# rishabhjain16/audio-visual-llm

Hardware: AMD Instinct MI355X
Metric: AV-clip train-step samples/sec (clip_whisper -> Llama-2-7B LoRA), whole job (higher is better)
Workload: dtype bf16

## Files before the change

audio-visual-llm_amd/csrc/api.hip:

```cpp
#include "common.h"
#include "avllm_internal.h"
#include <stdarg.h>

static thread_local char g_err[512] = "";

int av_set_error(int code, const char* fmt, ...) {
    va_list ap;
    va_start(ap, fmt);
    vsnprintf(g_err, sizeof(g_err), fmt, ap);
    va_end(ap);
    return code;
}

#include <mutex>
#include <string.h>
static const struct { const char* name; int dflt; } g_knob_def[AV_KNOB_COUNT] = {
    {"DECODE_FUSED", 1}, {"DEC_AL", 0}, {"LORA_UNBATCHED", 0}, {"F8_UNFUSED_QUANT", 0}, {"F8_FAST", 1}, {"ATTN_SHORT", 1},
    {"NARROW_EPILOGUE", 0}, {"TN_CHUNK", 0}, {"GEMM_DBG", 0}, {"GEMM_GW", 0}, {"GEMM_VARIANT", 0}};
static int g_knob[AV_KNOB_COUNT];
static std::once_flag g_knob_once;
static void knob_init() {
    for (int i = 0; i < AV_KNOB_COUNT; ++i) {
        char env[64];
        snprintf(env, sizeof(env), "AVLLM_%s", g_knob_def[i].name);
        const char* e = getenv(env);
        g_knob[i] = e ? atoi(e) : g_knob_def[i].dflt;
    }
}
int av_knob(int id) {
    std::call_once(g_knob_once, knob_init);
    return g_knob[id];
}
static int* knob_slot(const char* name) {
    std::call_once(g_knob_once, knob_init);
    for (int i = 0; name && i < AV_KNOB_COUNT; ++i)
        if (!strcmp(name, g_knob_def[i].name)) return &g_knob[i];
    return nullptr;
}

int av_device(int* ncu) {
    static int g_ncu[AV_MAX_DEVICES];
    int dev = 0;
    if (hipGetDevice(&dev) != hipSuccess) dev = 0;
    const int slot = dev & (AV_MAX_DEVICES - 1);
    if (!g_ncu[slot] && hipDeviceGetAttribute(&g_ncu[slot], hipDeviceAttributeMultiprocessorCount, dev) != hipSuccess) g_ncu[slot] = 256;
    *ncu = g_ncu[slot];
    return slot;
}

#define ST ((hipStream_t)stream)
extern "C" {
int avllm_set_knob(const char* name, int32_t value) {
    int* k = knob_slot(name);
    AV_CHECK_ARG(k, "set_knob: unknown knob '%s'", name ? name : "(null)");
    *k = value;
    return AV_OK;
}
int avllm_get_knob(const char* name, int32_t* value) {
    const int* k = knob_slot(name);
    AV_CHECK_ARG(k && value, "get_knob: unknown knob '%s'", name ? name : "(null)");
    *value = *k;
    return AV_OK;
}
int avllm_set_gemm_variant(int v) { return avllm_set_knob("GEMM_VARIANT", v); }
const char* avllm_last_error(void) { return g_err; }
int avllm_version(void) { return 100; }

int avllm_gemm(const avllm_gemm_desc* d, void* stream) { return av_gemm(d, ST); }
int avllm_gemm_plan(const avllm_gemm_desc* d, int32_t* kernel) { AV_CHECK_ARG(kernel, "gemm_plan: null kernel"); return av_gemm_plan(d, kernel); }
int avllm_gemm_tn(const void* P, int64_t ldp, int32_t I, const void* Q, int64_t ldq, int32_t J, int32_t M, float* out,
                  int64_t ldo, float alpha, int32_t dtype, void* stream) { return av_gemm_tn(P, ldp, I, Q, ldq, J, M, out, ldo, alpha, dtype, ST); }
int avllm_gemm_tn_drop(const void* P, int64_t ldp, int32_t I, const void* Q, int64_t ldq, int32_t J, int32_t M, float* out,
                       int64_t ldo, float alpha, uint32_t seed, float p, int32_t dtype, void* stream) { return av_gemm_tn(P, ldp, I, Q, ldq, J, M, out, ldo, alpha, dtype, ST, seed, p); }
int avllm_layernorm(const void* x, const void* w, const void* b, void* y, int64_t rows, int32_t d, float eps, int32_t dtype,
                    void* stream) { return av_layernorm(x, w, b, y, rows, d, eps, dtype, ST); }
int avllm_rmsnorm_fwd(const void* x, const void* w, void* y, float* rstd, int64_t rows, int32_t d, float eps, int32_t dtype,
                      void* stream) { return av_rmsnorm_fwd(x, w, y, rstd, rows, d, eps, dtype, ST); }
int avllm_rmsnorm_bwd(const void* dy, const void* x, const void* w, const float* rstd, const void* dres_in, void* dx_out,
                      int64_t rows, int32_t d, int32_t dtype, void* stream) { return av_rmsnorm_bwd(dy, x, w, rstd, dres_in, dx_out, rows, d, dtype, ST); }
int avllm_rope(void* x, int64_t ld, int64_t rows, int32_t T, int32_t heads, int32_t hd, int32_t pos0, float theta,
               int32_t inverse, int32_t dtype, void* stream) { return av_rope(x, ld, rows, T, heads, hd, pos0, theta, inverse, dtype, ST); }
int avllm_rope_table(float* tab, int32_t T, int32_t hd, int32_t pos0, float theta, const int32_t* pos_dev, float factor,
                     float low_freq_factor, float high_freq_factor, int32_t orig_ctx, void* stream) {
    AvRopeScale sc;
    sc.factor = factor; sc.low_freq_factor = low_freq_factor; sc.high_freq_factor = high_freq_factor; sc.orig_ctx = orig_ctx;
    AV_CHECK_ARG(orig_ctx <= 0 || (factor > 0.f && low_freq_factor > 0.f && high_freq_factor > low_freq_factor), "rope_table: bad llama3 scaling");
    return av_rope_table(tab, T, hd, pos0, theta, ST, pos_dev, sc);
}
int avllm_rope_tab(void* x, int64_t ld, int64_t rows, int32_t T, int32_t heads, int32_t hd, const float* tab, int32_t inverse,
                   int32_t dtype, void* stream) { return av_rope_tab(x, ld, rows, T, heads, hd, tab, inverse, dtype, ST); }
int avllm_kv_append(const void* k, const void* v, int64_t ld, void* kc, void* vc, int32_t B, int32_t T, int32_t pos0, int32_t Tmax,
                    int32_t d, int32_t dtype, void* stream) { return av_kv_append(k, v, ld, kc, vc, B, T, pos0, Tmax, d, dtype, ST); }
int avllm_swiglu_fwd(const void* gu, void* h, int64_t M, int32_t F, int32_t dtype, void* stream) { return av_swiglu_fwd(gu, h, M, F, dtype, ST); }
int avllm_swiglu_bwd(const void* dh, const void* gu, void* dgu, int64_t M, int32_t F, int32_t dtype, void* stream) { return av_swiglu_bwd(dh, gu, dgu, M, F, dtype, ST); }
int avllm_attention_fwd(const void* q, const void* k, const void* v, void* o, float* lse, int32_t B, int32_t Tq, int32_t Tk,
                        int32_t H, int32_t hd, int64_t ldq, int64_t ldk, int64_t ldv, int64_t ldo, float scale, int32_t causal,
                        int32_t dtype, int32_t impl, int32_t kv_heads, void* stream) {
    return av_attention_fwd(q, k, v, o, lse, B, Tq, Tk, H, hd, ldq, ldk, ldv, ldo, scale, causal, dtype, impl, ST, kv_heads);
}
int avllm_attention_bwd(const void* q, const void* k, const void* v, const void* o, const void* dout, const float* lse, void* dq,
                        void* dk, void* dv, float* delta_ws, int32_t B, int32_t T, int32_t H, int32_t hd, int64_t ldq, int64_t ldk,
                        int64_t ldv, int64_t ldo, int64_t lddq, int64_t lddk, int64_t lddv, float scale, int32_t causal,
                        int32_t dtype, int32_t impl, int32_t kv_heads, void* stream) {
    return av_attention_bwd(q, k, v, o, dout, lse, dq, dk, dv, delta_ws, B, T, H, hd, ldq, ldk, ldv, ldo, lddq, lddk, lddv, scale, causal, dtype, impl, ST, kv_heads);
}
int avllm_ce_fwd(const void* logits, int64_t ld, const int64_t* labels, int32_t B, int32_t T, int32_t V, float* row_lse,
                 float* loss_sum, float* count, int32_t dtype, void* stream) { return av_ce_fwd(logits, ld, labels, B, T, V, row_lse, loss_sum, count, dtype, ST); }
int avllm_ce_bwd(const void* logits, int64_t ld, const int64_t* labels, const float* row_lse, const float* count, float grad_scale,
                 void* dlogits, int32_t B, int32_t T, int32_t V, int32_t dtype, void* stream) { return av_ce_bwd(logits, ld, labels, row_lse, count, grad_scale, dlogits, B, T, V, dtype, ST); }
int avllm_argmax_rows(const void* logits, int64_t ld, int64_t rows, int32_t V, int64_t* out, int32_t dtype, void* stream) { return av_argmax_rows(logits, ld, rows, V, out, dtype, ST); }
int avllm_sample_rows(const void* logits, int64_t ld, int64_t rows, int32_t V, float temperature, int32_t top_k, float top_p, uint32_t seed,
                      const uint32_t* row_seeds, int32_t step, const int32_t* step_dev, uint8_t* unfinished, int64_t eos, int64_t pad,
                      int64_t* out, int32_t dtype, void* stream) {
    return av_sample_rows(logits, ld, rows, V, temperature, top_k, top_p, seed, row_seeds, step, step_dev, unfinished, eos, pad, out, dtype, ST);
}
size_t avllm_beam_topk_workspace_bytes(int64_t rows, int32_t V, int32_t k) { return av_beam_topk_workspace_bytes(rows, V, k); }
int avllm_beam_topk(const float* logits, int64_t ld, int32_t B, int32_t num_beams, int32_t V, const float* beam_scores, int32_t k,
                    float* out_scores, int32_t* out_beams, int64_t* out_tokens, void* ws, size_t ws_bytes, void* stream) {
    return av_beam_topk(logits, ld, B, num_beams, V, beam_scores, k, out_scores, out_beams, out_tokens, ws, ws_bytes, 0, ST);
}
int avllm_beam_topk_logprobs(const float* logprobs, int64_t ld, int32_t B, int32_t num_beams, int32_t V, const float* beam_scores, int32_t k,
                             float* out_scores, int32_t* out_beams, int64_t* out_tokens, void* ws, size_t ws_bytes, void* stream) {
    return av_beam_topk(logprobs, ld, B, num_beams, V, beam_scores, k, out_scores, out_beams, out_tokens, ws, ws_bytes, 1, ST);
}
int avllm_logits_process(void* scores, int64_t ld, int64_t rows, int32_t V, int64_t* history, int64_t ldh, const int64_t* append, int32_t cur,
                         const int32_t* cur_dev, float repetition_penalty, int32_t no_repeat_ngram_size, int32_t min_new_tokens, int64_t eos,
                         int32_t log_softmax, int32_t dtype, void* stream) {
    return av_logits_process(scores, ld, rows, V, history, ldh, append, cur, cur_dev, repetition_penalty, no_repeat_ngram_size, min_new_tokens, eos,
                             log_softmax, dtype, ST);
}
int avllm_kv_gather_rows(const void* k_src, const void* v_src, int32_t src_rows, int64_t src_T, void* k_dst, void* v_dst, int32_t dst_rows,
                         int64_t dst_T, int32_t layers, int32_t dkv, const int32_t* parent, int32_t t0, int32_t t1, int32_t dtype, void* stream) {
    return av_kv_gather_rows(k_src, v_src, src_rows, src_T, k_dst, v_dst, dst_rows, dst_T, layers, dkv, parent, t0, t1, dtype, ST);
}
int avllm_embedding(const void* table, const int64_t* ids, void* out, int64_t n, int32_t d, int32_t dtype, void* stream) { return av_embedding(table, ids, out, n, d, dtype, ST); }
int avllm_cast(const void* src, int32_t sdt, void* dst, int32_t ddt, int64_t n, void* stream) { return av_cast(src, sdt, dst, ddt, n, ST); }
int avllm_dropout(const void* x, void* y, int64_t rows, int32_t d, uint32_t seed, float p, int32_t dtype, void* stream) { return av_dropout(x, y, rows, d, seed, p, dtype, ST); }
int avllm_whisper_im2col1(const float* mel, void* cols, int32_t B, int32_t n_mels, int32_t T, int32_t Kpad, int32_t dtype, void* stream) { return av_whisper_im2col1(mel, cols, B, n_mels, T, Kpad, dtype, ST); }
int avllm_whisper_im2col2(const void* h, void* cols, int32_t B, int32_t T, int32_t d, int32_t dtype, void* stream) { return av_whisper_im2col2(h, cols, B, T, d, dtype, ST); }
int avllm_clip_patchify(const float* frames, void* cols, int32_t N, int32_t S, int32_t p, int32_t Kpad, int32_t dtype, void* stream) { return av_clip_patchify(frames, cols, N, S, p, Kpad, dtype, ST); }
int avllm_clip_cls_rows(const void* ce, const void* pos, void* x, int32_t N, int32_t tokens, int32_t d, int32_t dtype, void* stream) { return av_clip_cls_rows(ce, pos, x, N, tokens, d, dtype, ST); }
int avllm_fuse_pool(const void* a, int32_t Ta, const void* v, int32_t Tv, const void* pe, int32_t P, void* out, int32_t B, int32_t L,
                    int32_t S_out, int32_t D, float fs, int32_t dtype, void* stream) { return av_fuse_pool(a, Ta, v, Tv, pe, P, out, B, L, S_out, D, fs, dtype, ST); }
int avllm_fuse_pool_bwd(const void* dx, void* da, int32_t Ta, void* dv, int32_t Tv, int32_t P, int32_t B, int32_t L, int32_t S_out, int32_t D,
                        float fs, int32_t dtype, void* stream) { return av_fuse_pool_bwd(dx, da, Ta, dv, Tv, P, B, L, S_out, D, fs, dtype, ST); }
int avllm_gemm_wgrad(const void* dY, int64_t ldy, const void* X, int64_t ldx, int32_t M, int32_t N, int32_t K, float* dW, int64_t ldw, float* db,
                     float alpha, int32_t dtype, void* stream) { return av_gemm_wgrad(dY, ldy, X, ldx, M, N, K, dW, ldw, db, alpha, dtype, ST); }
int avllm_grad_sumsq_det_multi(const float* const* g, const int64_t* n, int32_t nbuf, float* partials, int32_t nparts, float* sumsq, void* stream) {
    return av_grad_sumsq_det_multi(g, n, nbuf, partials, nparts, sumsq, ST);
}
int avllm_adamw_step_multi(const avllm_adamw_seg* segs, int32_t nseg, float lr, float b1, float b2, float eps, int32_t step, const float* sumsq,
                           float max_norm, float prescale, const float* guard, float* skipped, const avllm_step_state* state, void* stream) {
    return av_adamw_step_multi(segs, nseg, lr, b1, b2, eps, step, sumsq, max_norm, prescale, guard, skipped, state, ST);
}
int avllm_grad_sumsq(const float* g, int64_t n, float* sumsq, void* stream) { return av_grad_sumsq(g, n, sumsq, ST); }
int avllm_grad_sumsq_det(const float* g, int64_t n, float* partials, int32_t nparts, float* sumsq, void* stream) { return av_grad_sumsq_det(g, n, partials, nparts, sumsq, ST); }
int avllm_adamw_step(float* p, const float* g, float* m, float* v, int64_t n, float lr, float b1, float b2, float eps, float wd,
                     int32_t step, const float* sumsq, float max_norm, float prescale, const float* guard, float* skipped,
                     const avllm_step_state* state, void* stream) {
    return av_adamw_step(p, g, m, v, n, lr, b1, b2, eps, wd, step, sumsq, max_norm, prescale, guard, skipped, state, ST);
}
int avllm_act_residual(const void* x, const void* r, void* y, int64_t n, int32_t act, int32_t dtype, void* stream) { return av_act_residual(x, r, y, n, act, dtype, ST); }
int avllm_step_advance(avllm_step_state* state, const avllm_schedule* sched, void* stream) { return av_step_advance(state, sched, ST); }
int avllm_lora_pack(const float* A, const float* Bm, int32_t r, int32_t din, int32_t dout, void* A_pad, void* AT_pad, int64_t ld_at,
                    void* B_pad, void* BT_pad, int32_t dtype, void* stream) { return av_lora_pack(A, Bm, r, din, dout, A_pad, AT_pad, ld_at, B_pad, BT_pad, dtype, ST); }
}
```

audio-visual-llm_amd/csrc/attention.hip:

```cpp
#include "common.h"
#include "avllm_internal.h"
#include <type_traits>
#include <cstdlib>

int av_attention_fwd_ref(const void* q, const void* k, const void* v, void* o, float* lse, int B, int Tq, int Tk, int H,
                         int hd, long ldq, long ldk, long ldv, long ldo, float scale, int causal, int dtype, hipStream_t st, int G);
int av_attention_delta(const void* o, const void* dout, float* delta, int B, int T, int H, int hd, long ldo, long lddo, int dtype, hipStream_t st);
int av_attention_bwd_ref(const void* q, const void* k, const void* v, const void* dout, const float* lse, const float* delta,
                         void* dq, void* dk, void* dv, int B, int T, int H, int hd, long ldq, long ldk, long ldv, long lddo,
                         long lddq, long lddk, long lddv, float scale, int causal, int dtype, hipStream_t st, int G);
int av_attention_bwd_mfma(const void* q, const void* k, const void* v, const void* dout, const float* lse, float* delta,
                          void* dq, void* dk, void* dv, int B, int T, int H, int hd, long ldq, long ldk, long ldv, long lddo,
                          long lddq, long lddk, long lddv, float scale, int causal, hipStream_t st, int G, const void* o, long ldo, const float* rope_tab);

namespace {

typedef __attribute__((address_space(3))) short4v* lds_s4_ptr;

__device__ __forceinline__ int acc_row(int reg, int half) { return (reg & 3) + 8 * (reg >> 2) + 4 * half; }
__device__ __forceinline__ float max3f(float a, float x, float y) { return __builtin_elementwise_maximum(__builtin_elementwise_maximum(a, x), y); }

template <int HD, int NW, bool CAUSAL>
__global__ __launch_bounds__(NW * 64, 2) void attn_fwd_mfma(const bf16* __restrict__ q, const bf16* __restrict__ k,
                                                         const bf16* __restrict__ v, bf16* __restrict__ o, float* __restrict__ lse,
// ... 75 lines not shown
            }
        }
        __syncthreads();
    }
    auto park = [&](int buf) {
#pragma unroll
        for (int i = 0; i < NCH; ++i) {
            const int c = tid + i * NT;
            if (c < 64 * CPR) {
                const int row = c / CPR, ch = c % CPR;
                *(u32x4*)(k_lds_ + buf * LROWS * KS + row * KS + ch * 16) = kreg[i];
                *(u32x4*)(v_lds_ + buf * LROWS * VS + row * VS + ch * 16) = vreg[i];
            }
        }
    };
    if (PREFETCH) prefetch(0);
    if (DB) { park(0); if (64 < k_end) prefetch(64); }
    for (int kb = 0; kb < k_end; kb += 64) {
        const int lrow0 = ONESHOT ? kb : 0;
        if (DB) {
            const int buf = (kb >> 6) & 1;
            __syncthreads();
            if (kb + 64 < k_end) { park(buf ^ 1); if (kb + 128 < k_end) prefetch(kb + 128); }
            k_lds = k_lds_ + buf * LROWS * KS; v_lds = v_lds_ + buf * LROWS * VS;
        } else if (!ONESHOT) {
            if (!PREFETCH) prefetch(kb);
            __syncthreads();
#pragma unroll
            for (int i = 0; i < NCH; ++i) {
                const int c = tid + i * NT;
                if (c < 64 * CPR) {
                    const int row = c / CPR, ch = c % CPR;
                    *(u32x4*)(k_lds + row * KS + ch * 16) = kreg[i];
                    *(u32x4*)(v_lds + row * VS + ch * 16) = vreg[i];
                }
            }
            __syncthreads();
            if (PREFETCH && kb + 64 < k_end) prefetch(kb + 64);
        }
        if (!wave_active || kb > wave_kmax) continue;

        const bool two = (kb + 32 <= wave_kmax) && (kb + 32 < Tk);
        f32x16 s0, s1;
#pragma unroll
        for (int i = 0; i < 16; ++i) { s0[i] = 0.f; s1[i] = 0.f; }
#pragma unroll
        for (int ks = 0; ks < HD / 16; ++ks) {
            const bf16x8 kf0 = *(const bf16x8*)(k_lds + (lrow0 + r) * KS + (2 * ks + half) * 16);
            s0 = __builtin_amdgcn_mfma_f32_32x32x16_bf16(kf0, qf[ks], s0, 0, 0, 0);
        }
        if (two) {
#pragma unroll
            for (int ks = 0; ks < HD / 16; ++ks) {
                const bf16x8 kf1 = *(const bf16x8*)(k_lds + (lrow0 + 32 + r) * KS + (2 * ks + half) * 16);
                s1 = __builtin_amdgcn_mfma_f32_32x32x16_bf16(kf1, qf[ks], s1, 0, 0, 0);
            }
        }
        const int klim = CAUSAL ? min(Tk - 1, qpos + off) : Tk - 1;
        const bool need_mask = (kb + 64 > Tk) || !two || (CAUSAL && kb + 63 > q0 + off);
        float mloc = -INFINITY;
        if (need_mask) {
#pragma unroll
            for (int i = 0; i < 16; ++i) {
                const int key0 = kb + acc_row(i, half);
                s0[i] = key0 <= klim ? s0[i] : -INFINITY;
                s1[i] = (two && key0 + 32 <= klim) ? s1[i] : -INFINITY;
            }
        }
#pragma unroll
        for (int i = 0; i < 16; ++i) mloc = max3f(mloc, s0[i], s1[i]);
        mloc = __builtin_elementwise_maximum(mloc, __shfl_xor(mloc, 32));
        mloc *= scale_log2e;
        const float m_new = __builtin_elementwise_maximum(m_run, mloc);
        const float m_use = m_new == -INFINITY ? 0.f : m_new;
        const float alpha = __builtin_amdgcn_exp2f(m_run - m_use);
        float psum = 0.f;
#pragma unroll
        for (int i = 0; i < 16; ++i) {
            s0[i] = __builtin_amdgcn_exp2f(fmaf(s0[i], scale_log2e, -m_use));
            s1[i] = __builtin_amdgcn_exp2f(fmaf(s1[i], scale_log2e, -m_use));
            psum += s0[i] + s1[i];
        }
        l_run = l_run * alpha + psum;
        m_run = m_new;
#pragma unroll
        for (int d = 0; d < HD / 32; ++d)
#pragma unroll
            for (int i = 0; i < 16; ++i) oacc[d][i] *= alpha;

        const int g = lane >> 4, i16 = lane & 15;
#pragma unroll
        for (int sb = 0; sb < 2; ++sb) {
            if (sb == 1 && !two) break;
#pragma unroll
            for (int s = 0; s < 2; ++s) {
                bf16x8 pb;
#pragma unroll
                for (int j = 0; j < 8; ++j) pb[j] = (bf16)(sb == 0 ? s0[8 * s + j] : s1[8 * s + j]);
                const int krow = lrow0 + 32 * sb + 16 * s + 4 * half + (i16 >> 2);
#pragma unroll
                for (int d = 0; d < HD / 32; ++d) {
                    const int col = 32 * d + 16 * (g & 1) + 4 * (i16 & 3);
                    const char* a0 = v_lds + krow * VS + col * 2;
                    const short4v lo = __builtin_amdgcn_ds_read_tr16_b64_v4i16((lds_s4_ptr)(a0));
                    const short4v hi = __builtin_amdgcn_ds_read_tr16_b64_v4i16((lds_s4_ptr)(a0 + 8 * VS));
                    typedef __attribute__((ext_vector_type(8))) short short8v;
                    const short8v both = {lo[0], lo[1], lo[2], lo[3], hi[0], hi[1], hi[2], hi[3]};
                    const bf16x8 vt = __builtin_bit_cast(bf16x8, both);
                    oacc[d] = __builtin_amdgcn_mfma_f32_32x32x16_bf16(vt, pb, oacc[d], 0, 0, 0);
                }
            }
        }
    }
    if (ONESHOT) {
        __syncthreads();
        const float l_tot = l_run + __shfl_xor(l_run, 32);
        const float inv = 1.0f / l_tot;
        char* ot = k_lds + w * 32 * KS;
#pragma unroll
        for (int d = 0; d < HD / 32; ++d)
#pragma unroll
            for (int g4 = 0; g4 < 4; ++g4) {
                float vals[4] = {oacc[d][4 * g4] * inv, oacc[d][4 * g4 + 1] * inv, oacc[d][4 * g4 + 2] * inv, oacc[d][4 * g4 + 3] * inv};
                store_f<4>((bf16*)(ot + r * KS) + 32 * d + 8 * g4 + 4 * half, vals);
            }
        if (lse && half == 0 && qpos < Tq) lse[((long)b * H + hh) * Tq + qpos] = (m_run + log2f(l_tot)) * 0.69314718055994531f;
        __builtin_amdgcn_wave_barrier();
        asm volatile("s_waitcnt lgkmcnt(0)" ::: "memory");
#pragma unroll
        for (int i = 0; i < 32 * CPR / 64; ++i) {
            const int c = lane + i * 64, row = c / CPR, ch = c % CPR;
            if (q0 + row < Tq)
                *(u32x4*)(o + ((long)b * Tq + q0 + row) * ldo + (long)hh * HD + ch * 8) = *(const u32x4*)(ot + row * KS + ch * 16);
        }
        return;
    }
    if (!wave_active) return;
    const float l_tot = l_run + __shfl_xor(l_run, 32);
    const float inv = 1.0f / l_tot;
    if (qpos < Tq) {
        bf16* op = o + ((long)b * Tq + qpos) * ldo + (long)hh * HD;
#pragma unroll
        for (int d = 0; d < HD / 32; ++d)
#pragma unroll
            for (int g4 = 0; g4 < 4; ++g4) {
                float vals[4] = {oacc[d][4 * g4] * inv, oacc[d][4 * g4 + 1] * inv, oacc[d][4 * g4 + 2] * inv, oacc[d][4 * g4 + 3] * inv};
                store_f<4>(op + 32 * d + 8 * g4 + 4 * half, vals);
            }
        if (lse && half == 0) lse[((long)b * H + hh) * Tq + qpos] = (m_run + log2f(l_tot)) * 0.69314718055994531f;
    }
}

template <int NKB, int NW, bool QOUT, bool FULLK>
__global__ __launch_bounds__(NW * 64) void attn_fwd_short(const bf16* __restrict__ q, const bf16* __restrict__ k, const bf16* __restrict__ v,
                                                          bf16* __restrict__ o, float* __restrict__ lse, int T, int H, long ldq, long ldk,
                                                          long ldv, long ldo, float scale_log2e, int G, uint8_t* __restrict__ oq, long ldoq,
                                                          uint8_t* __restrict__ osc, int RBo) {
    constexpr int HD = 64, KS = 160, VS = 160, OS = 80;
    constexpr int NPV = (NKB + 1) / 2, KROWS = NKB * 16, VROWS = NPV * 32, NT = NW * 64;
    constexpr int NQ = (NKB + NW - 1) / NW;
    extern __shared__ __attribute__((aligned(16))) char smem[];
    char* k_lds = smem;
    char* v_lds = smem + KROWS * KS;
    const int tid = threadIdx.x, lane = tid & 63, w = tid >> 6;
    char* o_lds = smem + KROWS * KS + VROWS * VS + w * 16 * OS;
    const int fr = lane & 15, fq = lane >> 4;
    const int hh = blockIdx.x, b = blockIdx.y, hk = hh / G;
    const int nkb = (T + 15) >> 4;

    constexpr int NCH = (VROWS * 8 + NT - 1) / NT;
    u32x4 kreg[NCH], vreg[NCH];
#pragma unroll
    for (int i = 0; i < NCH; ++i) {
        const int c = tid + i * NT, row = c >> 3, ch = c & 7;
        kreg[i] = (u32x4){0u, 0u, 0u, 0u}; vreg[i] = (u32x4){0u, 0u, 0u, 0u};
        if (row < T) {
            kreg[i] = *(const u32x4*)(k + ((long)b * T + row) * ldk + (long)hk * HD + ch * 8);
            vreg[i] = *(const u32x4*)(v + ((long)b * T + row) * ldv + (long)hk * HD + ch * 8);
        }
    }
    bf16x8 qf[NQ][2];
#pragma unroll
    for (int i = 0; i < NQ; ++i) {
        int qrow = (w + NW * i) * 16 + fr;
        qrow = qrow < T ? qrow : T - 1;
        const bf16* qp = q + ((long)b * T + qrow) * ldq + (long)hh * HD + 8 * fq;
        qf[i][0] = *(const bf16x8*)qp;
        qf[i][1] = *(const bf16x8*)(qp + 32);
    }
#pragma unroll
    for (int i = 0; i < NCH; ++i) {
        const int c = tid + i * NT, row = c >> 3, ch = c & 7;
        if (row < KROWS) *(u32x4*)(k_lds + row * KS + ch * 16) = kreg[i];
        if (row < VROWS) *(u32x4*)(v_lds + row * VS + ch * 16) = vreg[i];
    }
    __syncthreads();

    bf16x8 ones;
#pragma unroll
    for (int j = 0; j < 8; ++j) ones[j] = (bf16)1.0f;
    asm volatile("" : "+v"(ones));
    const f32x4 zero4 = {0.f, 0.f, 0.f, 0.f};
    const int i16 = lane & 15, g = lane >> 4;
    auto max3 = [](float a, float x, float y) __attribute__((always_inline)) { return max3f(a, x, y); };
    auto qblock = [&](int qi, auto fullc) __attribute__((always_inline)) {
        constexpr bool FULL = decltype(fullc)::value;
        const int qb = w + NW * qi;
        const int q0 = qb * 16;
        f32x4 sc[NKB];
#pragma unroll
        for (int kb = 0; kb < NKB; ++kb) {
            sc[kb] = (f32x4){-INFINITY, -INFINITY, -INFINITY, -INFINITY};
            if (FULL || kb < nkb) {
                const char* kr = k_lds + (kb * 16 + fr) * KS + fq * 16;
                const bf16x8 k0 = *(const bf16x8*)kr, k1 = *(const bf16x8*)(kr + 64);
                f32x4 a = __builtin_amdgcn_mfma_f32_16x16x32_bf16(k0, qf[qi][0], zero4, 0, 0, 0);
                sc[kb] = __builtin_amdgcn_mfma_f32_16x16x32_bf16(k1, qf[qi][1], a, 0, 0, 0);
            }
        }
        if (T & 15) {
            if constexpr (FULL) {
#pragma unroll
                for (int i = 0; i < 4; ++i) sc[NKB - 1][i] = ((NKB - 1) * 16 + 4 * fq + i < T) ? sc[NKB - 1][i] : -INFINITY;
            } else {
                const int kb = nkb - 1;
#pragma unroll
                for (int x = 0; x < NKB; ++x)
                    if (x == kb) {
#pragma unroll
                        for (int i = 0; i < 4; ++i) sc[x][i] = (x * 16 + 4 * fq + i < T) ? sc[x][i] : -INFINITY;
                    }
            }
        }
        float m = -INFINITY;
#pragma unroll
        for (int kb = 0; kb < NKB; ++kb) { m = max3(m, sc[kb][0], sc[kb][1]); m = max3(m, sc[kb][2], sc[kb][3]); }
        m = max3(m, __shfl_xor(m, 16), m);
        m = max3(m, __shfl_xor(m, 32), m);
        const float msc = m * scale_log2e;
        f32x4 lacc = zero4, oacc[4] = {zero4, zero4, zero4, zero4};
#pragma unroll
        for (int st = 0; st < NPV; ++st) {
            if (FULL || 2 * st < nkb) {
                bf16x8 pb;
                const bool second = 2 * st + 1 < NKB;
                const f32x4 s1 = sc[second ? 2 * st + 1 : 2 * st];
#pragma unroll
                for (int i = 0; i < 4; ++i) {
                    pb[i] = (bf16)__builtin_amdgcn_exp2f(fmaf(sc[2 * st][i], scale_log2e, -msc));
                    pb[4 + i] = second ? (bf16)__builtin_amdgcn_exp2f(fmaf(s1[i], scale_log2e, -msc)) : (bf16)0.f;
                }
                lacc = __builtin_amdgcn_mfma_f32_16x16x32_bf16(ones, pb, lacc, 0, 0, 0);
                const char* vr = v_lds + (32 * st + 4 * g + (i16 >> 2)) * VS + (4 * (i16 & 3)) * 2;
#pragma unroll
                for (int t = 0; t < 4; ++t) {
                    const short4v lo = __builtin_amdgcn_ds_read_tr16_b64_v4i16((lds_s4_ptr)(vr + t * 32));
                    const short4v hi = __builtin_amdgcn_ds_read_tr16_b64_v4i16((lds_s4_ptr)(vr + t * 32 + 16 * VS));
                    typedef __attribute__((ext_vector_type(8))) short short8v;
                    const short8v both = {lo[0], lo[1], lo[2], lo[3], hi[0], hi[1], hi[2], hi[3]};
                    oacc[t] = __builtin_amdgcn_mfma_f32_16x16x32_bf16(__builtin_bit_cast(bf16x8, both), pb, oacc[t], 0, 0, 0);
                }
            }
        }
        const float l = lacc[0], inv = 1.0f / l;
        if (lse && fq == 0 && q0 + fr < T) lse[((long)b * H + hh) * T + q0 + fr] = (msc + log2f(l)) * 0.69314718055994531f;
#pragma unroll
        for (int hf = 0; hf < 2; ++hf) {
#pragma unroll
            for (int tt = 0; tt < 2; ++tt) {
                const f32x4 a = oacc[2 * hf + tt];
                float vals[4] = {a[0] * inv, a[1] * inv, a[2] * inv, a[3] * inv};
                store_f<4>((bf16*)(o_lds + fr * OS) + 16 * tt + 4 * fq, vals);
            }
            asm volatile("s_waitcnt lgkmcnt(0)" ::: "memory");
            const int row = lane >> 2, ch = lane & 3;
            const u32x4 val = *(const u32x4*)(o_lds + row * OS + ch * 16);
            if constexpr (QOUT) {
                const bf16x8 vb = __builtin_bit_cast(bf16x8, val);
                float f[8], amax = 0.f;
#pragma unroll
                for (int c = 0; c < 8; ++c) { f[c] = (float)vb[c]; amax = fmaxf(amax, fabsf(f[c])); }
                amax = fmaxf(amax, __shfl_xor(amax, 1));
                amax = fmaxf(amax, __shfl_xor(amax, 2));
                int e = (int)((__float_as_uint(amax) >> 23) & 0xff) - 127 - 8;
                e = e < -127 ? -127 : (e > 127 ? 127 : e);
                const float invs = __uint_as_float((uint32_t)(127 - e) << 23);
#pragma unroll
                for (int c = 0; c < 8; ++c) f[c] = fminf(fmaxf(f[c] * invs, -448.f), 448.f);
                int r0 = 0, r1 = 0;
                r0 = __builtin_amdgcn_cvt_pk_fp8_f32(f[0], f[1], r0, false);
                r0 = __builtin_amdgcn_cvt_pk_fp8_f32(f[2], f[3], r0, true);
                r1 = __builtin_amdgcn_cvt_pk_fp8_f32(f[4], f[5], r1, false);
                r1 = __builtin_amdgcn_cvt_pk_fp8_f32(f[6], f[7], r1, true);
                if (q0 + row < T) {
                    const long m = (long)b * T + q0 + row;
                    typedef __attribute__((ext_vector_type(2))) unsigned int u32x2;
                    *(u32x2*)(oq + m * ldoq + (long)hh * HD + hf * 32 + ch * 8) = (u32x2){(uint32_t)r0, (uint32_t)r1};
                    if (ch == 0) {
                        const int cb = hh * (HD / 32) + hf;
                        osc[((((long)(cb >> 2) * RBo + (m >> 6)) * 4 + (cb & 3)) * 16 + (m & 15)) * 4 + ((m >> 4) & 3)] = (uint8_t)(e + 127);
                    }
                }
            } else {
                if (q0 + row < T) *(u32x4*)(o + ((long)b * T + q0 + row) * ldo + (long)hh * HD + hf * 32 + ch * 8) = val;
            }
            asm volatile("s_waitcnt lgkmcnt(0)" ::: "memory");
        }
    };
    if constexpr (FULLK) {
#pragma unroll
        for (int qi = 0; qi < NQ; ++qi)
            if (w + NW * qi < NKB) qblock(qi, std::true_type{});
    } else {
#pragma unroll
        for (int qi = 0; qi < NQ; ++qi)
            if (w + NW * qi < nkb) qblock(qi, std::false_type{});
    }
}

template <int NKB, int NW>
int launch_fwd_short(const void* q, const void* k, const void* v, void* o, float* lse, int B, int T, int H, long ldq, long ldk, long ldv,
                     long ldo, float scale, hipStream_t st, int G, void* oq = nullptr, long ldoq = 0, void* osc = nullptr) {
    constexpr int LDS = NKB * 16 * 160 + ((NKB + 1) / 2) * 32 * 160 + NW * 16 * 80;
    static bool attr[64] = {};
    int dev = 0;
    AV_HIP(hipGetDevice(&dev));
    if (!attr[dev & 63]) {
        AV_HIP(hipFuncSetAttribute((const void*)attn_fwd_short<NKB, NW, false, false>, hipFuncAttributeMaxDynamicSharedMemorySize, LDS));
        AV_HIP(hipFuncSetAttribute((const void*)attn_fwd_short<NKB, NW, true, false>, hipFuncAttributeMaxDynamicSharedMemorySize, LDS));
        AV_HIP(hipFuncSetAttribute((const void*)attn_fwd_short<NKB, NW, false, true>, hipFuncAttributeMaxDynamicSharedMemorySize, LDS));
        AV_HIP(hipFuncSetAttribute((const void*)attn_fwd_short<NKB, NW, true, true>, hipFuncAttributeMaxDynamicSharedMemorySize, LDS));
        attr[dev & 63] = true;
    }
    const int RBo = (int)(((long)B * T + 255) / 256 * 4);
    const bool fullk = ((T + 15) >> 4) == NKB;
#define AV_SHORT(QV, FV, OQ, LDOQ, OSC, RB) hipLaunchKernelGGL((attn_fwd_short<NKB, NW, QV, FV>), dim3(H, B), dim3(NW * 64), LDS, st, (const bf16*)q, (const bf16*)k, \
        (const bf16*)v, (bf16*)o, lse, T, H, ldq, ldk, ldv, ldo, scale * 1.4426950408889634f, G, OQ, LDOQ, OSC, RB)
    if (oq) { if (fullk) AV_SHORT(true, true, (uint8_t*)oq, ldoq, (uint8_t*)osc, RBo); else AV_SHORT(true, false, (uint8_t*)oq, ldoq, (uint8_t*)osc, RBo); }
    else { if (fullk) AV_SHORT(false, true, nullptr, 0, nullptr, 0); else AV_SHORT(false, false, nullptr, 0, nullptr, 0); }
#undef AV_SHORT
    AV_LAUNCH_CHECK();
    return AV_OK;
}

template <int HD, int NW>
int launch_fwd(const void* q, const void* k, const void* v, void* o, float* lse, int B, int Tq, int Tk, int H, long ldq,
               long ldk, long ldv, long ldo, float scale, int causal, hipStream_t st, int G) {
    const dim3 grid(av_cdiv(Tq, 32 * NW), H, B), block(NW * 64);
    const float sl = scale * 1.4426950408889634f;
    if (causal) hipLaunchKernelGGL((attn_fwd_mfma<HD, NW, true>), grid, block, 0, st, (const bf16*)q, (const bf16*)k, (const bf16*)v, (bf16*)o, lse, Tq, Tk, H, ldq, ldk, ldv, ldo, sl, G);
    else hipLaunchKernelGGL((attn_fwd_mfma<HD, NW, false>), grid, block, 0, st, (const bf16*)q, (const bf16*)k, (const bf16*)v, (bf16*)o, lse, Tq, Tk, H, ldq, ldk, ldv, ldo, sl, G);
    AV_LAUNCH_CHECK();
    return AV_OK;
}

}

int av_attention_fwd(const void* q, const void* k, const void* v, void* o, float* lse, int B, int Tq, int Tk, int H,
                     int hd, long ldq, long ldk, long ldv, long ldo, float scale, int causal, int dtype, int impl,
                     hipStream_t st, int kv_heads) {
    AV_CHECK_ARG(q && k && v && o && B > 0 && Tq > 0 && Tk > 0 && H > 0, "attention_fwd: bad args");
    if (kv_heads <= 0) kv_heads = H;
    AV_CHECK_ARG(H % kv_heads == 0, "attention_fwd: %d query heads are not a multiple of %d key/value heads", H, kv_heads);
    const int G = H / kv_heads;
    AV_CHECK_ARG(ldq % 8 == 0 && ldk % 8 == 0 && ldv % 8 == 0 && ldo % 8 == 0, "attention_fwd: row strides must be multiples of 8");
    AV_CHECK_ARG(!causal || Tk >= Tq, "attention_fwd: causal needs Tk >= Tq");
    if (impl == 1 || dtype == AV_F32 || (hd != 64 && hd != 128))
        return av_attention_fwd_ref(q, k, v, o, lse, B, Tq, Tk, H, hd, ldq, ldk, ldv, ldo, scale, causal, dtype, st, G);
    if (hd == 64) {
        const bool short_off = av_knob(AV_KNOB_ATTN_SHORT) == 0;
        if (!causal && Tq == Tk && !short_off && B <= 65535) {
            if (Tq <= 208) return launch_fwd_short<13, 7>(q, k, v, o, lse, B, Tq, H, ldq, ldk, ldv, ldo, scale, st, G);
            if (Tq <= 272) return launch_fwd_short<17, 9>(q, k, v, o, lse, B, Tq, H, ldq, ldk, ldv, ldo, scale, st, G);
        }
        if (Tq <= 224 && Tq > 128 && Tk <= 224 && !causal) return launch_fwd<64, 7>(q, k, v, o, lse, B, Tq, Tk, H, ldq, ldk, ldv, ldo, scale, causal, st, G);
        return launch_fwd<64, 4>(q, k, v, o, lse, B, Tq, Tk, H, ldq, ldk, ldv, ldo, scale, causal, st, G);
    }
    return launch_fwd<128, 4>(q, k, v, o, lse, B, Tq, Tk, H, ldq, ldk, ldv, ldo, scale, causal, st, G);
}

bool av_attention_fwd_mxq_ok(int B, int T, int H, int hd, int dtype, int kv_heads) {
    return dtype == AV_BF16 && hd == 64 && T <= 272 && B <= 65535 && (kv_heads <= 0 || kv_heads == H) && (H * hd) % 128 == 0 && av_knob(AV_KNOB_ATTN_SHORT) != 0 &&
           !av_knob(AV_KNOB_F8_UNFUSED_QUANT);
}
int av_attention_fwd_mxq(const void* q, const void* k, const void* v, void* oq, long ldoq, void* osc, int B, int T, int H, int hd, long ldq, long ldk,
                         long ldv, float scale, hipStream_t st) {
    AV_CHECK_ARG(q && k && v && oq && osc && av_attention_fwd_mxq_ok(B, T, H, hd, AV_BF16, H) && ldoq % 16 == 0 && ldq % 8 == 0 && ldk % 8 == 0 && ldv % 8 == 0,
                 "attention_fwd_mxq: bad args (bf16, head_dim 64, T <= 272, 16-byte aligned code rows)");
    if (T <= 208) return launch_fwd_short<13, 7>(q, k, v, nullptr, nullptr, B, T, H, ldq, ldk, ldv, 0, scale, st, 1, oq, ldoq, osc);
    return launch_fwd_short<17, 9>(q, k, v, nullptr, nullptr, B, T, H, ldq, ldk, ldv, 0, scale, st, 1, oq, ldoq, osc);
}
extern "C" int avllm_attention_fwd_mxq(const void* q, const void* k, const void* v, void* oq, int64_t ldoq, void* scales, int32_t B, int32_t T, int32_t H,
                                       int32_t hd, int64_t ldq, int64_t ldk, int64_t ldv, float scale, void* stream) {
    return av_attention_fwd_mxq(q, k, v, oq, ldoq, scales, B, T, H, hd, ldq, ldk, ldv, scale, (hipStream_t)stream);
}

bool av_attention_bwd_fuses_rope(int dtype, int hd, int impl) { return impl == 0 && dtype == AV_BF16 && (hd == 128 || hd == 64); }

int av_attention_bwd(const void* q, const void* k, const void* v, const void* o, const void* dout, const float* lse,
                     void* dq, void* dk, void* dv, float* delta_ws, int B, int T, int H, int hd, long ldq, long ldk,
                     long ldv, long ldo, long lddq, long lddk, long lddv, float scale, int causal, int dtype, int impl,
                     hipStream_t st, int kv_heads, const float* rope_tab) {
    AV_CHECK_ARG(q && k && v && o && dout && lse && dq && dk && dv && delta_ws, "attention_bwd: null");
    AV_CHECK_ARG(!rope_tab || av_attention_bwd_fuses_rope(dtype, hd, impl), "attention_bwd: the fused inverse RoPE exists in the bf16 MFMA kernels only");
    if (kv_heads <= 0) kv_heads = H;
    AV_CHECK_ARG(H % kv_heads == 0, "attention_bwd: %d query heads are not a multiple of %d key/value heads", H, kv_heads);
    const int G = H / kv_heads;
    if (impl == 0 && dtype == AV_BF16 && (hd == 128 || hd == 64))
        return av_attention_bwd_mfma(q, k, v, dout, lse, delta_ws, dq, dk, dv, B, T, H, hd, ldq, ldk, ldv, ldo, lddq, lddk, lddv, scale, causal, st, G, o, ldo, rope_tab);
    AV_TRY(av_attention_delta(o, dout, delta_ws, B, T, H, hd, ldo, ldo, dtype, st));
    return av_attention_bwd_ref(q, k, v, dout, lse, delta_ws, dq, dk, dv, B, T, H, hd, ldq, ldk, ldv, ldo, lddq, lddk, lddv, scale, causal, dtype, st, G);
}
```

audio-visual-llm_amd/csrc/common.h:

```cpp
#pragma once
#include <cstdlib>
#include <hip/hip_runtime.h>
#include <stdint.h>
#include <stdio.h>
#include <math.h>

typedef __bf16 bf16;
typedef __attribute__((ext_vector_type(2))) __bf16 bf16x2;
typedef __attribute__((ext_vector_type(4))) __bf16 bf16x4;
typedef __attribute__((ext_vector_type(8))) __bf16 bf16x8;
typedef __attribute__((ext_vector_type(4))) short short4v;
typedef __attribute__((ext_vector_type(2))) float f32x2;
typedef __attribute__((ext_vector_type(4))) float f32x4;
typedef __attribute__((ext_vector_type(16))) float f32x16;
typedef __attribute__((ext_vector_type(4))) unsigned int u32x4;

#define AV_WAVE 64

enum AvKnob { AV_KNOB_DECODE_FUSED, AV_KNOB_DEC_AL, AV_KNOB_LORA_UNBATCHED, AV_KNOB_F8_UNFUSED_QUANT, AV_KNOB_F8_FAST, AV_KNOB_ATTN_SHORT,
              AV_KNOB_NARROW_EPILOGUE, AV_KNOB_TN_CHUNK, AV_KNOB_GEMM_DBG, AV_KNOB_GEMM_GW, AV_KNOB_GEMM_VARIANT, AV_KNOB_COUNT };
int av_knob(int id);

#define AV_OK 0
#define AV_ERR_ARG 1
#define AV_ERR_HIP 2
#define AV_ERR_WORKSPACE 3
#define AV_ERR_UNSUPPORTED 4

extern "C" const char* avllm_last_error(void);
int av_set_error(int code, const char* fmt, ...);

#define AV_CHECK_ARG(cond, ...) \
    do { if (!(cond)) return av_set_error(AV_ERR_ARG, __VA_ARGS__); } while (0)
#define AV_HIP(expr) \
    do { hipError_t e_ = (expr); if (e_ != hipSuccess) return av_set_error(AV_ERR_HIP, "%s failed: %s (%s:%d)", #expr, hipGetErrorString(e_), __FILE__, __LINE__); } while (0)
#define AV_LAUNCH_CHECK() AV_HIP(hipGetLastError())
#define AV_TRY(expr) do { int rc_ = (expr); if (rc_ != AV_OK) return rc_; } while (0)

enum { AV_F32 = 0, AV_BF16 = 1 };
enum { AV_ACT_NONE = 0, AV_ACT_GELU = 1, AV_ACT_QUICK_GELU = 2, AV_ACT_SILU = 3 };

static inline size_t av_dtype_size(int dt) { return dt == AV_F32 ? 4 : 2; }

template <typename T> struct Vec;

__device__ __forceinline__ float to_f(float x) { return x; }
__device__ __forceinline__ float to_f(bf16 x) { return (float)x; }
template <typename T> __device__ __forceinline__ T from_f(float x);
template <> __device__ __forceinline__ float from_f<float>(float x) { return x; }
template <> __device__ __forceinline__ bf16 from_f<bf16>(float x) { return (bf16)x; }

template <typename T, int N> struct Pack { T v[N]; };

template <int N> __device__ __forceinline__ void load_f(const float* p, float (&o)[N]) {
    static_assert(N % 4 == 0, "");
#pragma unroll
    for (int i = 0; i < N; i += 4) { f32x4 t = *(const f32x4*)(p + i); o[i] = t[0]; o[i + 1] = t[1]; o[i + 2] = t[2]; o[i + 3] = t[3]; }
}
template <int N> __device__ __forceinline__ void load_f(const bf16* p, float (&o)[N]) {
    static_assert(N % 4 == 0, "");
    if constexpr (N % 8 == 0) {
#pragma unroll
        for (int i = 0; i < N; i += 8) { bf16x8 t = *(const bf16x8*)(p + i);
#pragma unroll
            for (int j = 0; j < 8; ++j) o[i + j] = (float)t[j]; }
    } else {
#pragma unroll
        for (int i = 0; i < N; i += 4) { bf16x4 t = *(const bf16x4*)(p + i);
#pragma unroll
            for (int j = 0; j < 4; ++j) o[i + j] = (float)t[j]; }
    }
}
template <int N> __device__ __forceinline__ void store_f(float* p, const float (&o)[N]) {
#pragma unroll
    for (int i = 0; i < N; i += 4) { f32x4 t = {o[i], o[i + 1], o[i + 2], o[i + 3]}; *(f32x4*)(p + i) = t; }
}
template <int N> __device__ __forceinline__ void store_f(bf16* p, const float (&o)[N]) {
    if constexpr (N % 8 == 0) {
#pragma unroll
        for (int i = 0; i < N; i += 8) { bf16x8 t;
#pragma unroll
            for (int j = 0; j < 8; ++j) t[j] = (bf16)o[i + j];
            *(bf16x8*)(p + i) = t; }
    } else {
#pragma unroll
        for (int i = 0; i < N; i += 4) { bf16x4 t;
#pragma unroll
            for (int j = 0; j < 4; ++j) t[j] = (bf16)o[i + j];
            *(bf16x4*)(p + i) = t; }
    }
}

__device__ __forceinline__ float wave_sum(float v) {
#pragma unroll
    for (int o = 32; o > 0; o >>= 1) v += __shfl_xor(v, o);
    return v;
}
__device__ __forceinline__ float wave_max(float v) {
#pragma unroll
    for (int o = 32; o > 0; o >>= 1) v = fmaxf(v, __shfl_xor(v, o));
    return v;
}
__device__ __forceinline__ float block_sum(float v, float* red) {
    v = wave_sum(v);
    const int w = threadIdx.x >> 6, nw = (blockDim.x + 63) >> 6;
    __syncthreads();
    if ((threadIdx.x & 63) == 0) red[w] = v;
    __syncthreads();
    float t = 0.f;
    for (int i = 0; i < nw; ++i) t += red[i];
    return t;
}
__device__ __forceinline__ float block_max(float v, float* red) {
    v = wave_max(v);
    const int w = threadIdx.x >> 6, nw = (blockDim.x + 63) >> 6;
    __syncthreads();
    if ((threadIdx.x & 63) == 0) red[w] = v;
    __syncthreads();
    float t = -INFINITY;
    for (int i = 0; i < nw; ++i) t = fmaxf(t, red[i]);
    return t;
}

__device__ __forceinline__ float act_apply(float x, int act) {
    switch (act) {
        case AV_ACT_GELU: return 0.5f * x * (1.0f + erff(x * 0.70710678118654752f));
        case AV_ACT_QUICK_GELU: return x / (1.0f + __expf(-1.702f * x));
        case AV_ACT_SILU: return x / (1.0f + __expf(-x));
        default: return x;
    }
}
__device__ __forceinline__ float act_apply_fast(float x, int act) {
    switch (act) {
        case AV_ACT_GELU: {
            const float z = fabsf(x) * 0.70710678118654752f;
            const float t = __builtin_amdgcn_rcpf(1.0f + 0.3275911f * z);
            const float poly = t * (0.254829592f + t * (-0.284496736f + t * (1.421413741f + t * (-1.453152027f + t * 1.061405429f))));
            const float erf_abs = 1.0f - poly * __builtin_amdgcn_exp2f(-z * z * 1.4426950408889634f);
            return 0.5f * x * (1.0f + copysignf(erf_abs, x));
        }
        case AV_ACT_QUICK_GELU: return x * __builtin_amdgcn_rcpf(1.0f + __builtin_amdgcn_exp2f(-1.702f * 1.4426950408889634f * x));
        case AV_ACT_SILU: return x * __builtin_amdgcn_rcpf(1.0f + __builtin_amdgcn_exp2f(-1.4426950408889634f * x));
        default: return x;
    }
}

__host__ __device__ __forceinline__ uint32_t av_hash32(uint32_t x) {
    x ^= x >> 16; x *= 0x7feb352dU; x ^= x >> 15; x *= 0x846ca68bU; x ^= x >> 16;
    return x;
}
__host__ __device__ __forceinline__ uint32_t av_drop_thr(float p) { return (uint32_t)(p * 65536.0f); }
__host__ __device__ __forceinline__ float av_drop_scale(float p) { return 1.0f / (1.0f - (float)av_drop_thr(p) * (1.0f / 65536.0f)); }
__host__ __device__ __forceinline__ uint32_t av_pair_hash(uint32_t seed, unsigned long long pair) {
    const uint32_t hi = (uint32_t)(pair >> 32);
    uint32_t inner = av_hash32(seed);
    if (__builtin_expect(hi != 0u, 0)) inner = av_hash32(seed + hi * 0x9E3779B9U);
    return av_hash32((uint32_t)pair ^ inner);
}
__host__ __device__ __forceinline__ bool av_keep(uint32_t seed, unsigned long long idx, float p) {
    const uint32_t h = av_pair_hash(seed, idx >> 1);
    return ((idx & 1) ? (h >> 16) : (h & 0xffffu)) >= av_drop_thr(p);
}
__device__ __forceinline__ uint32_t av_seed(const uint32_t* seed_dev, uint32_t off) { return (seed_dev ? *seed_dev : 0u) + off; }
__device__ __forceinline__ void av_mask8(float (&v)[8], uint32_t seed, unsigned long long idx0, uint32_t thr, float sc) {
    const unsigned long long p0 = idx0 >> 1;
    if (__builtin_expect(((p0 + 3) >> 32) == 0, 1)) {
        const uint32_t inner = av_hash32(seed);
#pragma unroll
        for (int q = 0; q < 4; ++q) {
            const uint32_t h = av_hash32(((uint32_t)p0 + q) ^ inner);
            v[2 * q] = (h & 0xffffu) >= thr ? v[2 * q] * sc : 0.f;
            v[2 * q + 1] = (h >> 16) >= thr ? v[2 * q + 1] * sc : 0.f;
        }
// ... 12 lines not shown
```

Baseline: 93.61.

## Make short attention forward persistent with prefetch of next head's K/V/Q

Turns the short-sequence attention forward kernel into a persistent kernel: the grid is sized to CUs times resident blocks, and each workgroup loops over (batch, head) items. While computing the current item it issues global loads for the next item's K/V inside the PV loop and its Q after each query block, hiding load latency behind MFMA work. It also sets a minimum-occupancy launch bound and removes the B<=65535 limit. The risks are register pressure from the prefetch registers and occupancy bounds, and more complex control flow.

```diff
diff --git a/audio-visual-llm_amd/csrc/api.hip b/audio-visual-llm_amd/csrc/api.hip
--- a/audio-visual-llm_amd/csrc/api.hip
+++ b/audio-visual-llm_amd/csrc/api.hip
@@ -16,7 +16,8 @@
 #include <string.h>
 static const struct { const char* name; int dflt; } g_knob_def[AV_KNOB_COUNT] = {
     {"DECODE_FUSED", 1}, {"DEC_AL", 0}, {"LORA_UNBATCHED", 0}, {"F8_UNFUSED_QUANT", 0}, {"F8_FAST", 1}, {"ATTN_SHORT", 1},
-    {"NARROW_EPILOGUE", 0}, {"TN_CHUNK", 0}, {"GEMM_DBG", 0}, {"GEMM_GW", 0}, {"GEMM_VARIANT", 0}};
+    {"NARROW_EPILOGUE", 0}, {"TN_CHUNK", 0}, {"GEMM_DBG", 0}, {"GEMM_GW", 0}, {"GEMM_VARIANT", 0},
+    {"ATTN_SHORT_GRID", 0}};
 static int g_knob[AV_KNOB_COUNT];
 static std::once_flag g_knob_once;
 static void knob_init() {
diff --git a/audio-visual-llm_amd/csrc/attention.hip b/audio-visual-llm_amd/csrc/attention.hip
--- a/audio-visual-llm_amd/csrc/attention.hip
+++ b/audio-visual-llm_amd/csrc/attention.hip
@@ -251,10 +251,10 @@
 }
 
 template <int NKB, int NW, bool QOUT, bool FULLK>
-__global__ __launch_bounds__(NW * 64) void attn_fwd_short(const bf16* __restrict__ q, const bf16* __restrict__ k, const bf16* __restrict__ v,
+__global__ __launch_bounds__(NW * 64, NKB <= 13 ? 4 : 3) void attn_fwd_short(const bf16* __restrict__ q, const bf16* __restrict__ k, const bf16* __restrict__ v,
                                                           bf16* __restrict__ o, float* __restrict__ lse, int T, int H, long ldq, long ldk,
                                                           long ldv, long ldo, float scale_log2e, int G, uint8_t* __restrict__ oq, long ldoq,
-                                                          uint8_t* __restrict__ osc, int RBo) {
+                                                          uint8_t* __restrict__ osc, int RBo, int items) {
     constexpr int HD = 64, KS = 160, VS = 160, OS = 80;
     constexpr int NPV = (NKB + 1) / 2, KROWS = NKB * 16, VROWS = NPV * 32, NT = NW * 64;
     constexpr int NQ = (NKB + NW - 1) / NW;
@@ -264,36 +264,39 @@
     const int tid = threadIdx.x, lane = tid & 63, w = tid >> 6;
     char* o_lds = smem + KROWS * KS + VROWS * VS + w * 16 * OS;
     const int fr = lane & 15, fq = lane >> 4;
-    const int hh = blockIdx.x, b = blockIdx.y, hk = hh / G;
     const int nkb = (T + 15) >> 4;
+    const int nkbx = FULLK ? NKB : nkb;
+    int it = blockIdx.x;
+    if (it >= items) return;
+    int b = it / H, hh = it - b * H;
+    int nb = b, nhh = hh;
+    bool more = false;
 
     constexpr int NCH = (VROWS * 8 + NT - 1) / NT;
+    constexpr int PF0 = (NKB <= 13 && QOUT) ? 2 : 1;
+    static_assert(PF0 + NCH < NPV, "prefetch steps");
     u32x4 kreg[NCH], vreg[NCH];
-#pragma unroll
-    for (int i = 0; i < NCH; ++i) {
-        const int c = tid + i * NT, row = c >> 3, ch = c & 7;
+    auto opaque = [](int x) __attribute__((always_inline)) { asm volatile("" : "+v"(x)); return x; };
+    auto kv_issue = [&](int t, int i, int bb, int hkk, bool on) __attribute__((always_inline)) {
+        const int c = t + i * NT, row = c >> 3, ch = c & 7;
         kreg[i] = (u32x4){0u, 0u, 0u, 0u}; vreg[i] = (u32x4){0u, 0u, 0u, 0u};
-        if (row < T) {
-            kreg[i] = *(const u32x4*)(k + ((long)b * T + row) * ldk + (long)hk * HD + ch * 8);
-            vreg[i] = *(const u32x4*)(v + ((long)b * T + row) * ldv + (long)hk * HD + ch * 8);
-        }
-    }
+        if (on && row < T) {
+            kreg[i] = *(const u32x4*)(k + ((long)bb * T + row) * ldk + (long)hkk * HD + ch * 8);
+            vreg[i] = *(const u32x4*)(v + ((long)bb * T + row) * ldv + (long)hkk * HD + ch * 8);
+        }
+    };
     bf16x8 qf[NQ][2];
-#pragma unroll
-    for (int i = 0; i < NQ; ++i) {
-        int qrow = (w + NW * i) * 16 + fr;
+    auto q_issue = [&](int t, int i, int bb, int hq) __attribute__((always_inline)) {
+        int qrow = ((t >> 6) + NW * i) * 16 + (t & 15);
         qrow = qrow < T ? qrow : T - 1;
-        const bf16* qp = q + ((long)b * T + qrow) * ldq + (long)hh * HD + 8 * fq;
+        const bf16* qp = q + ((long)bb * T + qrow) * ldq + (long)hq * HD + 8 * ((t >> 4) & 3);
         qf[i][0] = *(const bf16x8*)qp;
         qf[i][1] = *(const bf16x8*)(qp + 32);
-    }
-#pragma unroll
-    for (int i = 0; i < NCH; ++i) {
-        const int c = tid + i * NT, row = c >> 3, ch = c & 7;
-        if (row < KROWS) *(u32x4*)(k_lds + row * KS + ch * 16) = kreg[i];
-        if (row < VROWS) *(u32x4*)(v_lds + row * VS + ch * 16) = vreg[i];
-    }
-    __syncthreads();
+    };
+#pragma unroll
+    for (int i = 0; i < NCH; ++i) kv_issue(tid, i, b, hh / G, true);
+#pragma unroll
+    for (int i = 0; i < NQ; ++i) q_issue(tid, i, b, hh);
 
     bf16x8 ones;
 #pragma unroll
@@ -302,10 +305,11 @@
     const f32x4 zero4 = {0.f, 0.f, 0.f, 0.f};
     const int i16 = lane & 15, g = lane >> 4;
     auto max3 = [](float a, float x, float y) __attribute__((always_inline)) { return max3f(a, x, y); };
-    auto qblock = [&](int qi, auto fullc) __attribute__((always_inline)) {
+    auto qblock = [&](int qi, auto fullc, auto pfc) __attribute__((always_inline)) {
         constexpr bool FULL = decltype(fullc)::value;
-        const int qb = w + NW * qi;
-        const int q0 = qb * 16;
+        constexpr bool PF = decltype(pfc)::value;
+        const int tl = opaque(tid);
+        const int q0 = ((tl >> 6) + NW * qi) * 16;
         f32x4 sc[NKB];
 #pragma unroll
         for (int kb = 0; kb < NKB; ++kb) {
@@ -360,9 +364,10 @@
                     oacc[t] = __builtin_amdgcn_mfma_f32_16x16x32_bf16(__builtin_bit_cast(bf16x8, both), pb, oacc[t], 0, 0, 0);
                 }
             }
+            if (PF && st >= PF0 && st - PF0 < NCH) kv_issue(tl, st - PF0, nb, nhh / G, more);
         }
         const float l = lacc[0], inv = 1.0f / l;
-        if (lse && fq == 0 && q0 + fr < T) lse[((long)b * H + hh) * T + q0 + fr] = (msc + log2f(l)) * 0.69314718055994531f;
+        if (lse && (tl & 48) == 0 && q0 + (tl & 15) < T) lse[((long)b * H + hh) * T + q0 + (tl & 15)] = (msc + log2f(l)) * 0.69314718055994531f;
 #pragma unroll
         for (int hf = 0; hf < 2; ++hf) {
 #pragma unroll
@@ -372,7 +377,7 @@
                 store_f<4>((bf16*)(o_lds + fr * OS) + 16 * tt + 4 * fq, vals);
             }
             asm volatile("s_waitcnt lgkmcnt(0)" ::: "memory");
-            const int row = lane >> 2, ch = lane & 3;
+            const int ol = tl & 63, row = ol >> 2, ch = ol & 3;
             const u32x4 val = *(const u32x4*)(o_lds + row * OS + ch * 16);
             if constexpr (QOUT) {
                 const bf16x8 vb = __builtin_bit_cast(bf16x8, val);
@@ -406,14 +411,37 @@
             asm volatile("s_waitcnt lgkmcnt(0)" ::: "memory");
         }
     };
-    if constexpr (FULLK) {
-#pragma unroll
-        for (int qi = 0; qi < NQ; ++qi)
-            if (w + NW * qi < NKB) qblock(qi, std::true_type{});
-    } else {
-#pragma unroll
-        for (int qi = 0; qi < NQ; ++qi)
-            if (w + NW * qi < nkb) qblock(qi, std::false_type{});
+#pragma clang loop unroll(disable)
+    for (;;) {
+#pragma unroll
+        for (int i = 0; i < NCH; ++i) {
+            const int c = tid + i * NT, row = c >> 3, ch = c & 7;
+            if (row < KROWS) *(u32x4*)(k_lds + row * KS + ch * 16) = kreg[i];
+            if (row < VROWS) *(u32x4*)(v_lds + row * VS + ch * 16) = vreg[i];
+        }
+        __syncthreads();
+        {
+            const int nx = it + (int)gridDim.x;
+            more = nx < items;
+            if (more) { nb = nx / H; nhh = nx - nb * H; }
+        }
+        static_assert(NQ == 2, "two query blocks per wave at most");
+        constexpr std::integral_constant<bool, FULLK> fullc{};
+        if (w + NW < nkbx) {
+            qblock(0, fullc, std::false_type{});
+            if (more) q_issue(opaque(tid), 0, nb, nhh);
+            qblock(1, fullc, std::true_type{});
+            if (more) q_issue(opaque(tid), 1, nb, nhh);
+        } else if (w < nkbx) {
+            qblock(0, fullc, std::true_type{});
+            if (more) q_issue(opaque(tid), 0, nb, nhh);
+        } else {
+#pragma unroll
+            for (int i = 0; i < NCH; ++i) kv_issue(opaque(tid), i, nb, nhh / G, more);
+        }
+        if (!more) break;
+        it += (int)gridDim.x; b = nb; hh = nhh;
+        __syncthreads();
     }
 }
 
@@ -421,20 +449,27 @@
 int launch_fwd_short(const void* q, const void* k, const void* v, void* o, float* lse, int B, int T, int H, long ldq, long ldk, long ldv,
                      long ldo, float scale, hipStream_t st, int G, void* oq = nullptr, long ldoq = 0, void* osc = nullptr) {
     constexpr int LDS = NKB * 16 * 160 + ((NKB + 1) / 2) * 32 * 160 + NW * 16 * 80;
-    static bool attr[64] = {};
-    int dev = 0;
-    AV_HIP(hipGetDevice(&dev));
-    if (!attr[dev & 63]) {
+    static int resident[AV_MAX_DEVICES] = {};
+    int ncu = 0;
+    const int dev = av_device(&ncu);
+    if (!resident[dev]) {
         AV_HIP(hipFuncSetAttribute((const void*)attn_fwd_short<NKB, NW, false, false>, hipFuncAttributeMaxDynamicSharedMemorySize, LDS));
         AV_HIP(hipFuncSetAttribute((const void*)attn_fwd_short<NKB, NW, true, false>, hipFuncAttributeMaxDynamicSharedMemorySize, LDS));
         AV_HIP(hipFuncSetAttribute((const void*)attn_fwd_short<NKB, NW, false, true>, hipFuncAttributeMaxDynamicSharedMemorySize, LDS));
         AV_HIP(hipFuncSetAttribute((const void*)attn_fwd_short<NKB, NW, true, true>, hipFuncAttributeMaxDynamicSharedMemorySize, LDS));
-        attr[dev & 63] = true;
-    }
+        int per_cu = 0;
+        AV_HIP(hipOccupancyMaxActiveBlocksPerMultiprocessor(&per_cu, (const void*)attn_fwd_short<NKB, NW, true, true>, NW * 64, LDS));
+        resident[dev] = per_cu > 0 ? per_cu : 1;
+    }
+    const long items = (long)B * H;
+    AV_CHECK_ARG(items <= 0x7fffffffL - 65536, "attention_fwd: %ld (item, head) pairs", items);
+    const int cap = av_knob(AV_KNOB_ATTN_SHORT_GRID);
+    const long wgs = cap > 0 ? cap : (long)ncu * resident[dev];
+    const int grid = (int)(items < wgs ? items : wgs);
     const int RBo = (int)(((long)B * T + 255) / 256 * 4);
     const bool fullk = ((T + 15) >> 4) == NKB;
-#define AV_SHORT(QV, FV, OQ, LDOQ, OSC, RB) hipLaunchKernelGGL((attn_fwd_short<NKB, NW, QV, FV>), dim3(H, B), dim3(NW * 64), LDS, st, (const bf16*)q, (const bf16*)k, \
-        (const bf16*)v, (bf16*)o, lse, T, H, ldq, ldk, ldv, ldo, scale * 1.4426950408889634f, G, OQ, LDOQ, OSC, RB)
+#define AV_SHORT(QV, FV, OQ, LDOQ, OSC, RB) hipLaunchKernelGGL((attn_fwd_short<NKB, NW, QV, FV>), dim3(grid), dim3(NW * 64), LDS, st, (const bf16*)q, (const bf16*)k, \
+        (const bf16*)v, (bf16*)o, lse, T, H, ldq, ldk, ldv, ldo, scale * 1.4426950408889634f, G, OQ, LDOQ, OSC, RB, (int)items)
     if (oq) { if (fullk) AV_SHORT(true, true, (uint8_t*)oq, ldoq, (uint8_t*)osc, RBo); else AV_SHORT(true, false, (uint8_t*)oq, ldoq, (uint8_t*)osc, RBo); }
     else { if (fullk) AV_SHORT(false, true, nullptr, 0, nullptr, 0); else AV_SHORT(false, false, nullptr, 0, nullptr, 0); }
 #undef AV_SHORT
@@ -468,7 +503,7 @@
         return av_attention_fwd_ref(q, k, v, o, lse, B, Tq, Tk, H, hd, ldq, ldk, ldv, ldo, scale, causal, dtype, st, G);
     if (hd == 64) {
         const bool short_off = av_knob(AV_KNOB_ATTN_SHORT) == 0;
-        if (!causal && Tq == Tk && !short_off && B <= 65535) {
+        if (!causal && Tq == Tk && !short_off) {
             if (Tq <= 208) return launch_fwd_short<13, 7>(q, k, v, o, lse, B, Tq, H, ldq, ldk, ldv, ldo, scale, st, G);
             if (Tq <= 272) return launch_fwd_short<17, 9>(q, k, v, o, lse, B, Tq, H, ldq, ldk, ldv, ldo, scale, st, G);
         }
@@ -479,7 +514,7 @@
 }
 
 bool av_attention_fwd_mxq_ok(int B, int T, int H, int hd, int dtype, int kv_heads) {
-    return dtype == AV_BF16 && hd == 64 && T <= 272 && B <= 65535 && (kv_heads <= 0 || kv_heads == H) && (H * hd) % 128 == 0 && av_knob(AV_KNOB_ATTN_SHORT) != 0 &&
+    return dtype == AV_BF16 && hd == 64 && T <= 272 && (kv_heads <= 0 || kv_heads == H) && (H * hd) % 128 == 0 && av_knob(AV_KNOB_ATTN_SHORT) != 0 &&
            !av_knob(AV_KNOB_F8_UNFUSED_QUANT);
 }
 int av_attention_fwd_mxq(const void* q, const void* k, const void* v, void* oq, long ldoq, void* osc, int B, int T, int H, int hd, long ldq, long ldk,
diff --git a/audio-visual-llm_amd/csrc/common.h b/audio-visual-llm_amd/csrc/common.h
--- a/audio-visual-llm_amd/csrc/common.h
+++ b/audio-visual-llm_amd/csrc/common.h
@@ -18,7 +18,8 @@
 #define AV_WAVE 64
 
 enum AvKnob { AV_KNOB_DECODE_FUSED, AV_KNOB_DEC_AL, AV_KNOB_LORA_UNBATCHED, AV_KNOB_F8_UNFUSED_QUANT, AV_KNOB_F8_FAST, AV_KNOB_ATTN_SHORT,
-              AV_KNOB_NARROW_EPILOGUE, AV_KNOB_TN_CHUNK, AV_KNOB_GEMM_DBG, AV_KNOB_GEMM_GW, AV_KNOB_GEMM_VARIANT, AV_KNOB_COUNT };
+              AV_KNOB_NARROW_EPILOGUE, AV_KNOB_TN_CHUNK, AV_KNOB_GEMM_DBG, AV_KNOB_GEMM_GW, AV_KNOB_GEMM_VARIANT,
+              AV_KNOB_ATTN_SHORT_GRID, AV_KNOB_COUNT };
 int av_knob(int id);
 
 #define AV_OK 0
```

New measurement: 93.64 (median of 2 runs). About the same (+0.0%).
